# scttfrdmn/bwa-mem2-arm

Hardware: AMD Instinct MI355X
Metric: M seed-extensions/sec (150 bp, band=100) at 1/2/4/8 MI355X vs CPU (higher is better)
Workload: dtype int16; 1 GPU; C2: 1000000 SeqPairs/GPU resident in HBM, 150 bp query / 300 bp ref, band w=100, cell_bits=16, h0 U[19,100]; pairs_per_gpu=1000000, parallelism=shard1 (independent pairs), distinct_gpus=1

## Files before the change

bwa-mem2-arm_amd/csrc/bsw_dispatch.hip:

```cpp
#include <hip/hip_runtime.h>
#include <hipcub/hipcub.hpp>
#include <algorithm>
#include <cstring>
#include "bsw_engine.h"
#include <emmintrin.h>

namespace bsw {

constexpr int kNumLaneClasses = 5;
constexpr int kPkClass0 = kNumLaneClasses;
constexpr int kWideClass = kPkClass0 + kNumLaneClasses;
constexpr int kWvClass0 = kWideClass + 1;
constexpr int kNumWvClasses = 3;
constexpr int kWvCols[kNumWvClasses] = {4, 8, 16};
constexpr int kNumClasses = kWvClass0 + kNumWvClasses;
static_assert(kNumClasses <= kMetaCounts, "class counts");

__device__ __forceinline__ int seed_matches(const uint8_t *__restrict__ q, int qlen,
                                            const uint8_t *__restrict__ r, int tlen)
{
    if (qlen < 40 || tlen < 46) return 31;
    uint8_t qb[30], rb[42];
#pragma unroll
    for (int j = 0; j < 30; ++j) qb[j] = q[10 + j];
#pragma unroll
    for (int j = 0; j < 42; ++j) rb[j] = r[4 + j];
    int best = 0;
#pragma unroll
    for (int sft = 0; sft <= 12; ++sft) {
        int c = 0;
#pragma unroll
        for (int j = 0; j < 30; ++j) c += qb[j] == rb[j + sft];
        best = max(best, c);
    }
    return best;
}

__device__ __forceinline__ int wv_class(const KParams &kp, int32_t w, int qlen, int tlen, int h0)
{
    if (kp.maxsc != 1 || qlen > kWvQmax || h0 < 0) return -1;
    if ((int64_t)kp.e_ins * qlen >= 2700) return -1;
    if (128 + kp.o_del + 2 * kp.e_del >= 30000 || 128 + kp.o_ins + 2 * kp.e_ins >= 30000) return -1;
    if ((int64_t)h0 + min(qlen, tlen) + (int64_t)kp.e_ins * (qlen + 1) >= 30000) return -1;
    int wl = w;
    const int ni = qlen * kp.maxsc + kp.end_bonus - kp.o_ins;
    const int nd = qlen * kp.maxsc + kp.end_bonus - kp.o_del;
    wl = min(wl, max((ni + kp.e_ins) / kp.e_ins, 1));
    wl = min(wl, max((nd + kp.e_del) / kp.e_del, 1));
    for (int k = 0; k < kNumWvClasses; ++k)
        if (2 * wl + kWvCols[k] + 2 <= 64 * kWvCols[k]) return kWvClass0 + k;
    return -1;
}

__global__ void plan_kernel(const SeqPair *__restrict__ pairs, int32_t n, const KParams kp, int32_t w,
                            int32_t pc_route, int32_t wv_route, const uint8_t *__restrict__ ref,
                            const uint8_t *__restrict__ qer, uint32_t *__restrict__ keys,
                            int32_t *__restrict__ vals, int32_t *__restrict__ counts,
                            int32_t *__restrict__ maxq_wide, int keymode, int misroute)
{
    const int maxsc = kp.maxsc;
    const int i = blockIdx.x * blockDim.x + threadIdx.x;
    const bool valid = i < n;
    SeqPair p{};
    if (valid) p = pairs[i];
    const int qlen = max(p.len2, 0), tlen = max(p.len1, 0);
    const int64_t hi = (int64_t)max(p.h0, 0) + (int64_t)max(maxsc, 0) * min(qlen, tlen);
    int c = kWideClass;
    const int wvc = wv_route ? wv_class(kp, w, qlen, tlen, p.h0) : -1;
    if (wv_route == 2 && wvc >= 0) c = wvc;
    else if (hi < 32768 && p.h0 >= 0) {
        if (qlen <= 32) c = 0;
        else if (qlen <= 64) c = 1;
        else if (qlen <= 96) c = 2;
        else if (qlen <= 128) c = 3;
        else if (qlen <= 160) c = 4;
        if (pc_route && c < kNumLaneClasses && p.h0 + min(qlen, tlen) <= 255 && qlen + 1 <= 160)
            c = kPkClass0 + (qlen + 1 <= 32 ? 0 : qlen + 1 <= 64 ? 1 : qlen + 1 <= 96 ? 2 : qlen + 1 <= 128 ? 3 : 4);
    }
    if (c == kWideClass && wvc >= 0) c = wvc;
    if (misroute) c = 0;
    if (valid) {
        if (c == kWideClass) atomicMax(maxq_wide, qlen);
        const int mt = (c == kWideClass) ? 31 : seed_matches(qer + p.idq, qlen, ref + p.idr, tlen);
        const int rel = mt > 18;
        if (keymode == 0)
            keys[i] = ((uint32_t)c << 28) | ((uint32_t)(255 - min(qlen, 255)) << 20) |
                      ((uint32_t)(1 - rel) << 19) | ((uint32_t)(2047 - min(tlen, 2047)) << 8) |
                      (uint32_t)(255 - min(max(p.h0, 0), 255));
        else
            keys[i] = ((uint32_t)c << 28) | ((uint32_t)(255 - min(qlen, 255)) << 20) |
                      ((uint32_t)(1 - rel) << 19) | ((uint32_t)(63 - min(tlen >> 5, 63)) << 13) |
                      ((uint32_t)(31 - min(mt, 31)) << 8) | (uint32_t)(255 - min(max(p.h0, 0), 255));
        vals[i] = i;
    }
    __shared__ int s_cnt[kNumClasses];
    if (threadIdx.x < kNumClasses) s_cnt[threadIdx.x] = 0;
    __syncthreads();
    const int lane = threadIdx.x & 63;
#pragma unroll
// ... 126 lines not shown
        BSW_TRY(hipEventRecord(s.evh, pc.stream));
        BSW_TRY(hipStreamWaitEvent(stream, s.evh, 0));
    }
    BSW_TRY(grow_sort(s, n));
    BSW_TRY(hipMemsetAsync(s.d_meta, 0, kMetaWords * sizeof(int32_t), stream));
    int32_t *d_counts = s.d_meta, *d_maxq = s.d_meta + kMetaMaxq;
    const int pc_route = (kp.pk_ok && kp.kern8) ? 1 : 0;
    const int32_t long_route = (kp.long_route == 1 && n <= kp.small_batch) ? 2 : kp.long_route;
    hipLaunchKernelGGL(plan_kernel, dim3((unsigned)((n + 255) / 256)), dim3(256), 0, stream,
                       pc.d_pairs, n, kp, pc.w, pc_route, long_route, pc.d_ref, pc.d_qer, s.d_keys,
                       s.d_vals, d_counts, d_maxq, (int)kp.keymode, (int)kp.misroute);
    BSW_TRY(hipGetLastError());
    BSW_TRY(sort_order(s, n, kKeyBits, stream));
    BSW_TRY(hipMemcpyAsync(s.h_meta, s.d_meta, kMetaWords * sizeof(int32_t), hipMemcpyDeviceToHost, stream));
    if (!s.evm) BSW_TRY(hipEventCreateWithFlags(&s.evm.p, hipEventDisableTiming));
    BSW_TRY(hipEventRecord(s.evm, stream));
    return BSW_OK;
}

int run_dp(const KParams &kp, Slot &s)
{
    const PlanCall &pc = s.plan;
    if (pc.n == 0) return BSW_OK;
    hipStream_t stream = pc.dp_stream && !s.fast ? pc.dp_stream : pc.stream;
    const int32_t w = pc.w;
    const int cell_bits = pc.cell_bits;
    SeqPair *d_pairs = pc.d_pairs;
    const uint8_t *d_ref = pc.d_ref, *d_qer = pc.d_qer;
    int32_t *d_err = s.d_meta + kMetaErr;
    if (s.fast) {
        if (s.fast == 1) {
            BSW_TRY(hipEventSynchronize(s.evm));
            if (s.h_meta[kMetaFlag] != 0) {
                PlanCall again = pc;
                again.gq_maxq = -1;
                const int r = run_plan(kp, s, again);
                if (r) return r;
                return run_dp(kp, s);
            }
        }
        s.timed = true;
        return BSW_OK;
    }
    BSW_TRY(hipEventSynchronize(s.evm));
    BSW_TRY(hipStreamWaitEvent(stream, s.evm, 0));
    int32_t counts[kNumClasses] = {};
    for (int sl = 0; sl < kMetaSpread; ++sl)
        for (int c = 0; c < kNumClasses; ++c) counts[c] += s.h_meta[sl * kMetaCounts + c];
    const int32_t maxq_wide = s.h_meta[kMetaMaxq];
    int nclass = 0;
    for (int c = 0; c < kNumClasses; ++c) nclass += counts[c] > 0;
    const bool fork = nclass > 1 && kp.fork;
    BSW_TRY(hipEventRecord(s.ev0, stream));
    if (fork) {
        if (!s.evf) BSW_TRY(hipEventCreateWithFlags(&s.evf.p, hipEventDisableTiming));
        for (int k = 0; k < Slot::kSide; ++k)
            if (!s.side[k]) {
                BSW_TRY(hipStreamCreateWithFlags(&s.side[k].p, hipStreamNonBlocking));
                BSW_TRY(hipEventCreateWithFlags(&s.evj[k].p, hipEventDisableTiming));
            }
        BSW_TRY(hipEventRecord(s.evf, stream));
        for (int k = 0; k < Slot::kSide; ++k) BSW_TRY(hipStreamWaitEvent(s.side[k], s.evf, 0));
    }
    int nl = 0;
    auto next_stream = [&]() {
        const int k = nl++ % (1 + Slot::kSide);
        return (fork && k > 0) ? s.side[k - 1] : stream;
    };
    const int lrc = [&]() -> int {
        int32_t off = 0;
        for (int c = 0; c < kNumLaneClasses; ++c) {
            if (counts[c] > 0) {
                BSW_TRY(launch_lane_kernel(kLaneQmax[c], kp, w, d_pairs, s.d_order + off, counts[c],
                                           d_ref, d_qer, d_err, next_stream()));
                s.stats.n_launches++;
                s.stats.n_i16 += counts[c];
            }
            off += counts[c];
        }
        for (int c = 0; c < kNumLaneClasses; ++c) {
            const int32_t np = counts[kPkClass0 + c];
            if (np > 0) {
                BSW_TRY(launch_pc_kernel(kLaneQmax[c], kp, w, d_pairs, s.d_order + off, np, d_ref, d_qer,
                                         d_err, next_stream()));
                s.stats.n_launches++;
                s.stats.n_packed += np;
                if (cell_bits == 8) s.stats.n_u8 += np;
                else s.stats.n_i16 += np;
            }
            off += np;
        }
        if (counts[kWideClass] > 0) {
            const int32_t nw = counts[kWideClass];
            const size_t need = (size_t)(maxq_wide + 2) * (size_t)nw;
            BSW_TRY(s.d_scratch.grow(need));
            BSW_TRY(launch_wide_kernel(kp, w, d_pairs, s.d_order + off, nw, d_ref, d_qer, s.d_scratch,
                                       nw, next_stream()));
            s.stats.n_launches++;
            s.stats.n_wide += nw;
        }
        off += counts[kWideClass];
        for (int c = 0; c < kNumWvClasses; ++c) {
            const int32_t nv = counts[kWvClass0 + c];
            if (nv > 0) {
                BSW_TRY(launch_wv_kernel(kWvCols[c], kp, w, d_pairs, s.d_order + off, nv, d_ref, d_qer, d_err,
                                         next_stream()));
                s.stats.n_launches++;
                s.stats.n_i16 += nv;
                s.stats.n_wave += nv;
            }
            off += nv;
        }
        return BSW_OK;
    }();
    if (fork)
        for (int k = 0; k < Slot::kSide; ++k) {
            BSW_TRY(hipEventRecord(s.evj[k], s.side[k]));
            BSW_TRY(hipStreamWaitEvent(stream, s.evj[k], 0));
        }
    if (lrc) {
        (void)hipStreamSynchronize(stream);
        return lrc;
    }
    BSW_TRY(hipEventRecord(s.ev1, stream));
    BSW_TRY(hipMemcpyAsync(s.h_meta + kMetaErr, d_err, sizeof(int32_t), hipMemcpyDeviceToHost, stream));
    s.run_stream = stream;
    s.timed = true;
    return BSW_OK;
}

int run_device(const KParams &kp, Slot &s, SeqPair *d_pairs, const uint8_t *d_ref,
                      const uint8_t *d_qer, int32_t n, int32_t w, int cell_bits, hipStream_t stream)
{
    PlanCall pc;
    pc.d_pairs = d_pairs; pc.d_ref = d_ref; pc.d_qer = d_qer;
    pc.n = n; pc.w = w; pc.cell_bits = cell_bits; pc.stream = stream;
    int r = run_plan(kp, s, pc);
    if (r) return r;
    return run_dp(kp, s);
}

int finish_stats(Slot &s, bool spin)
{
    if (s.timed) {
        float ms = 0.f;
        s.timed = false;
        if (spin) {
            hipError_t q;
            while ((q = hipStreamQuery(s.run_stream)) == hipErrorNotReady) _mm_pause();
            BSW_TRY(q);
        }
        BSW_TRY(hipStreamSynchronize(s.run_stream));
        BSW_TRY(hipEventElapsedTime(&ms, s.ev0, s.ev1));
        s.stats.kernel_ms = ms;
        if (s.h_meta[kMetaErr] != 0) return BSW_E_RANGE;
    }
    return BSW_OK;
}

}
```

bwa-mem2-arm_amd/csrc/bsw_engine.h:

```cpp
#pragma once
#include <hip/hip_runtime.h>
#include <algorithm>
#include <atomic>
#include <condition_variable>
#include <cstdint>
#include <deque>
#include <memory>
#include <mutex>
#include <shared_mutex>
#include <type_traits>
#include <utility>
#include <vector>
#include "../../include/bsw.h"
#include "../../include/bsw_mate.h"
#include "../../include/bsw_global.h"
#include "../../include/bsw_aln.h"
#include "../../include/bsw_sel.h"
#include "../../include/bsw_pe.h"
#include "../../include/bsw_matesw.h"
#include "../../include/bsw_rec.h"
#include "../../include/bsw_contigs.h"
#include "bsw_contig_seg.h"
#include "bsw_kernels.h"
#include "bsw_internal.h"

#define BSW_HIDDEN __attribute__((visibility("hidden")))

namespace bsw {

constexpr int kMetaCounts = 16;
constexpr int kMetaSpread = 32;
constexpr int kMetaMaxq = kMetaCounts * kMetaSpread;
constexpr int kMetaErr = kMetaMaxq + 1;
constexpr int kMetaFlag = kMetaErr + 1;
constexpr int kMetaCnt = kMetaFlag + 1;
constexpr int kMetaWords = kMetaCnt + 1;
constexpr int kKeyBits = 32;
constexpr int32_t kStageBlk = 4096;

static inline int hip_rc(hipError_t e)
{
    if (e == hipSuccess) return BSW_OK;
    if (e == hipErrorOutOfMemory) return BSW_E_NOMEM;
    return BSW_E_HIP;
}
#define BSW_TRY(x) do { hipError_t _e = (x); if (_e != hipSuccess) return ::bsw::hip_rc(_e); } while (0)

BSW_HIDDEN bool inject_nomem();

template <class P, class Free>
struct BSW_HIDDEN Owned {
    P p = nullptr;
    Owned() = default;
    Owned(const Owned &) = delete;
    Owned &operator=(const Owned &) = delete;
    Owned(Owned &&o) noexcept : p(std::exchange(o.p, nullptr)) {}
    Owned &operator=(Owned &&o) noexcept { std::swap(p, o.p); return *this; }
    ~Owned() { reset(); }
    void reset() { if (p) (void)Free()(p); p = nullptr; }
    operator P() const { return p; }
};
struct BSW_HIDDEN FreeDev { hipError_t operator()(void *p) const { return hipFree(p); } };
struct BSW_HIDDEN FreeHost { hipError_t operator()(void *p) const { return hipHostFree(p); } };
struct BSW_HIDDEN FreeStream { hipError_t operator()(hipStream_t s) const { return hipStreamDestroy(s); } };
struct BSW_HIDDEN FreeEvent { hipError_t operator()(hipEvent_t e) const { return hipEventDestroy(e); } };
using Stream = Owned<hipStream_t, FreeStream>;
using Event = Owned<hipEvent_t, FreeEvent>;

template <class T, class Free>
struct BSW_HIDDEN Buf : Owned<T *, Free> {
    size_t cap = 0;
    Buf() = default;
    Buf(Buf &&o) noexcept : Owned<T *, Free>(std::move(o)), cap(std::exchange(o.cap, 0)) {}
    Buf &operator=(Buf &&o) noexcept { std::swap(this->p, o.p); std::swap(cap, o.cap); return *this; }
    void reset() { Owned<T *, Free>::reset(); cap = 0; }
    hipError_t reserve_exact(size_t n)
    {
        reset();
        hipError_t e;
        if constexpr (std::is_same<Free, FreeDev>::value) e = hipMalloc((void **)&this->p, n * sizeof(T));
        else e = hipHostMalloc((void **)&this->p, n * sizeof(T), 0);
        if (e == hipSuccess) cap = n;
        else this->p = nullptr;
        return e;
    }
    size_t grown(size_t need) const { return std::max(need + need / 4, cap * 3 / 2); }
};
template <class T>
struct BSW_HIDDEN DevBuf : Buf<T, FreeDev> {
    hipError_t grow(size_t need)
    {
        if (need <= this->cap) return hipSuccess;
        if (inject_nomem()) return hipErrorOutOfMemory;
        return this->reserve_exact(this->grown(need));
    }
};
template <class T>
struct BSW_HIDDEN PinnedBuf : Buf<T, FreeHost> {
    hipError_t grow(size_t need) { return need <= this->cap ? hipSuccess : this->reserve_exact(this->grown(need)); }
};

struct PlanCall {
    SeqPair *d_pairs = nullptr;
    const uint8_t *d_ref = nullptr, *d_qer = nullptr;
    int32_t n = 0, w = 0;
    int cell_bits = 16;
    hipStream_t stream = nullptr;
    hipStream_t dp_stream = nullptr;
    hipStream_t plan_stream = nullptr;
    int gq_maxq = -2, gq_maxt = 0;
    int32_t *d_out24 = nullptr;
};

struct ExtState;
struct AlnState;
struct SelW;
struct SelRd;
struct PeV;
struct MswSt;
// ... 262 lines not shown
```

bwa-mem2-arm_amd/csrc/bsw_kernels.h:

```cpp
#pragma once
#include <stdint.h>
#include <hip/hip_runtime.h>
#include "../../include/bsw_seqpair.h"

namespace bsw {

struct KParams {
    int32_t o_del, e_del, o_ins, e_ins;
    int32_t zdrop, end_bonus;
    int32_t maxsc;
    int32_t pk_ok;
    uint32_t prof[8][2];
    int8_t mat[25];
    int8_t kern8;
    int8_t keymode;
    int8_t fork;
    int8_t misroute;
    int8_t long_route;
    int8_t group_kernel;
    int32_t mid_batch;
    int32_t small_batch;
    int32_t gq32_max;
};

struct PairIn {
    int32_t idr, idq, len1, len2, h0;
};
static_assert(sizeof(PairIn) == 20, "PairIn");

constexpr int kLaneQmax[] = {32, 64, 96, 128, 160};
constexpr int kLaneQmaxMax = 160;

hipError_t launch_lane_kernel(int qmax, const KParams &kp, int32_t w, SeqPair *pairs,
                              const int32_t *order, int32_t n, const uint8_t *ref,
                              const uint8_t *qer, int32_t *err, hipStream_t s);

hipError_t launch_pc_kernel(int qmax, const KParams &kp, int32_t w, SeqPair *pairs,
                            const int32_t *order, int32_t n, const uint8_t *ref,
                            const uint8_t *qer, int32_t *err, hipStream_t s);

constexpr int kWvQmax = 4096;
hipError_t launch_wv_kernel(int cols, const KParams &kp, int32_t w, SeqPair *pairs, const int32_t *order,
                            int32_t n, const uint8_t *ref, const uint8_t *qer, int32_t *err, hipStream_t s);

hipError_t launch_gq_kernel(int gs, int cols, const KParams &kp, int32_t w, SeqPair *pairs, const int32_t *order,
                            int32_t n, const uint8_t *ref, const uint8_t *qer, int32_t *err, int32_t *flag,
                            int32_t *out24, hipStream_t s);
int gq_cols_for(int max_qlen, int gs);
bool gq_pair_ok(const KParams &kp, int qlen, int tlen, int h0, int gs);

hipError_t launch_wide_kernel(const KParams &kp, int32_t w, SeqPair *pairs,
                              const int32_t *order, int32_t n, const uint8_t *ref,
                              const uint8_t *qer, int2 *scratch, int32_t scratch_stride,
                              hipStream_t s);

}
```

bwa-mem2-arm_amd/csrc/bsw_pc.hip:

```cpp
#include <hip/hip_runtime.h>
#include <stdint.h>
#include <stdlib.h>
#include <limits.h>
#include <utility>
#include "bsw_kernels.h"
#include "bsw_wave.h"

namespace bsw {

constexpr int kPcChunkDw = 17;
#ifndef BSW_PC_EXP_HALFHEAD
#define BSW_PC_EXP_HALFHEAD 0
#endif
#ifdef BSW_PC_STATS
__device__ unsigned long long g_pc_stats[11];
constexpr int kPcTimesMax = 1 << 16;
__device__ unsigned long long g_pc_times[kPcTimesMax][4];
#endif

struct PcRow {
    uint64_t enter;
    uint64_t fast;
    uint64_t left;
};

__device__ __forceinline__ uint64_t gbits(int lo, int n)
{
    uint64_t m;
    asm("s_bfm_b64 %0, %1, %2" : "=s"(m)
        : "s"(__builtin_amdgcn_readfirstlane(min(n, 63))), "s"(__builtin_amdgcn_readfirstlane(lo)));
    return m;
}

__device__ __forceinline__ uint32_t pack2(int v) { return ((uint32_t)v & 0xffffu) * 0x10001u; }

#define PC_SDWA(op, d, a, b, sel) \
    op "_sdwa " d ", " a ", " b " dst_sel:DWORD dst_unused:UNUSED_PAD src0_sel:DWORD src1_sel:" sel "\n\t"

#define PC_PH1_(X, EOUT, ESUB)                                                          \
    "v_pk_min_i16 %[s" X "], %[s" X "], %[h" X "]\n\t"                                      \
    "v_pk_add_u16 %[s" X "], %[s" X "], %[h" X "]\n\t"                                      \
    "v_pk_sub_i16 %[t" X "], %[s" X "], %[oe2]\n\t"                                         \
    "v_pk_max_i16 %[s" X "], %[s" X "], %[e" X "]\n\t"                                      \
    ESUB                                                                                     \
    "v_pk_max_i16 " EOUT ", " EOUT ", %[t" X "]\n\t"
#define PC_PH1(X, EOUT) PC_PH1_(X, EOUT, "v_pk_sub_i16 " EOUT ", %[e" X "], %[ed2]\n\t")
#define PC_PH1B(X, EOUT) PC_PH1_(X, EOUT, "v_pk_sub_u16 " EOUT ", %[e" X "], %[ed2] clamp\n\t")

#define PC_SCORES                                                                        \
    "v_perm_b32 %[y], %[phi], %[plo], %[q]\n\t"                                              \
    "v_pk_lshlrev_b16 %[sa], 8, %[y] op_sel_hi:[0,1]\n\t"                                    \
    "v_pk_ashrrev_i16 %[sa], 8, %[sa] op_sel_hi:[0,1]\n\t"                                   \
    "v_pk_ashrrev_i16 %[sb], 8, %[y] op_sel_hi:[0,1]\n\t"

#define PC_CELL(C, X, W)                                                                 \
    PC_SDWA("v_max_i32", C, "%[f]", "sext(%[s" X "])", W)                                    \
    "v_subrev_u32_e64 %[f], %[ed], %[f] clamp\n\t"                                           \
    PC_SDWA("v_max_i32", "%[f]", "%[f]", "sext(%[t" X "])", W)

#define PC_RESET(HP, RJ)                                                                 \
    "v_cmp_ne_u32_e32 vcc, " RJ ", %[begv]\n\t"                                              \
    "v_cndmask_b32_e32 " HP ", 0, " HP ", vcc\n\t"                                           \
    "v_cndmask_b32_e32 %[f], 0, %[f], vcc\n\t"
#define PC_MCELL(C, HP, X, W, J)                                                         \
    PC_CELL(C, X, W)                                                                         \
    "v_cmp_lt_i32_e32 vcc, " J ", %[endv]\n\t"                                               \
    "v_cndmask_b32_e32 " C ", " HP ", " C ", vcc\n\t"

#define PC_MWRITE(X, KEYSRC, LEFT)                                                       \
    "v_pk_sub_i16 %[y], %[jj" X "], %[endw]\n\t"                                             \
    "v_pk_ashrrev_i16 %[y], 15, %[y] op_sel_hi:[0,1]\n\t"                                    \
    "v_bfi_b32 %[h" X "], %[y], %[p" X "], %[h" X "]\n\t"                                    \
    "v_bfi_b32 %[e" X "], %[y], 0, %[e" X "]\n\t"                                            \
    KEYSRC                                                                                   \
    "v_and_b32_e32 %[p" X "], %[p" X "], %[y]\n\t"                                           \
    "v_pk_sub_i16 %[y], %[jj" X "], %[endm1w]\n\t"                                           \
    "v_pk_ashrrev_i16 %[y], 15, %[y] op_sel_hi:[0,1]\n\t"                                    \
    "v_bfi_b32 %[e" X "], %[y], %[x" X "], %[e" X "]\n\t"                                    \
    LEFT                                                                                     \
    "v_pk_max_u16 %[key], %[key], %[p" X "]\n\t"
#define PC_LEFTMASK(X)                                                                   \
    "v_pk_sub_i16 %[y], %[begm2w], %[jj" X "]\n\t"                                           \
    "v_pk_ashrrev_i16 %[y], 15, %[y] op_sel_hi:[0,1]\n\t"                                    \
    "v_and_b32_e32 %[p" X "], %[p" X "], %[y]\n\t"

#define PC_MASKED(CH0, CH1, CH2, CH3, KA, KB, LA, LB) PC_MASKED_(PC_PH1, CH0, CH1, CH2, CH3, KA, KB, LA, LB)
#define PC_MASKED_(PH, CH0, CH1, CH2, CH3, KA, KB, LA, LB)                               \
    PH("a", "%[xa]") PH("b", "%[xb]")                                                        \
    CH0 CH1                                                                                  \
    "v_lshl_or_b32 %[pa], %[c0], 16, %[h1]\n\t"                                              \
    CH2 CH3                                                                                  \
    "v_lshl_or_b32 %[pb], %[c2], 16, %[c1]\n\t"                                              \
    PC_MWRITE("a", KA, LA) PC_MWRITE("b", KB, LB)

#ifdef BSW_PC_STATS
#define PC_CNT(k) "v_add_u32_e32 %[ct" #k "], 1, %[ct" #k "]\n\t"
#define PC_CNT_OPS , [ct0] "+v"(ctr[0]), [ct1] "+v"(ctr[1]), [ct2] "+v"(ctr[2]), [ct3] "+v"(ctr[3])
#else
// ... 345 lines not shown
        if constexpr (2 * GG + 1 < QMAX / 2) pc_lastpos_reg<2 * GG + 1>(hh[2 * GG + 1], endp1w, lp);
        pc_lastpos_reg<2 * GG>(hh[2 * GG], endp1w, lp);
    }
    return pending & (lp == 0u);
}

template <int QMAX, bool BY, int... G>
__device__ __forceinline__ int pc_lastpos(std::integer_sequence<int, G...>, const uint32_t (&hh)[(BY ? QMAX / 4 : QMAX / 2)],
                                          int end, bool need, int gstart)
{
    bool pending = need;
    uint32_t lp = 0;
    const uint32_t endp1w = pack2(end + 1);
    ((pending = pc_lastpos_group<QMAX, BY, QMAX / 4 - 1 - G>(hh, endp1w, pending, lp, gstart)), ...);
    return (int)max(lp & 0xffffu, lp >> 16);
}

#ifndef BSW_PC_EARLY_STOP
#define BSW_PC_EARLY_STOP 1
#endif
#ifndef BSW_PC_EARLY_SCAN
#define BSW_PC_EARLY_SCAN 1
#endif
#ifndef BSW_PC_SCAN_PHASE
#define BSW_PC_SCAN_PHASE 3
#endif

template <int K>
__device__ __forceinline__ void pc_ub_reg(uint32_t hv, uint32_t qw, uint32_t begw, uint32_t &ub)
{
    constexpr uint32_t SC = (uint32_t)(2 * K) | ((uint32_t)(2 * K + 1) << 16);
    uint32_t c, m;
    asm volatile(
        "v_pk_sub_i16 %[c], %[qw], %[sc]\n\t"
        "v_pk_ashrrev_i16 %[m], 15, %[c] op_sel_hi:[0,1]\n\t"
        "v_pk_add_u16 %[c], %[c], %[h]\n\t"
        "v_bfi_b32 %[c], %[m], 0, %[c]\n\t"
        "v_pk_sub_i16 %[m], %[bg], %[sc]\n\t"
        "v_pk_ashrrev_i16 %[m], 15, %[m] op_sel_hi:[0,1]\n\t"
        "v_and_b32_e32 %[c], %[c], %[m]\n\t"
        "v_pk_max_u16 %[ub], %[ub], %[c]\n\t"
        : [ub] "+v"(ub), [c] "=&v"(c), [m] "=&v"(m)
        : [h] "v"(hv), [qw] "v"(qw), [sc] "s"(SC), [bg] "v"(begw));
}

template <int QMAX, bool BY, int GG>
__device__ __forceinline__ void pc_ub_group(const uint32_t (&hh)[(BY ? QMAX / 4 : QMAX / 2)], uint32_t qw,
                                            uint32_t begw, uint32_t &ub, uint64_t enter)
{
    if (!((enter >> GG) & 1)) return;
    if constexpr (BY) {
        pc_ub_reg<2 * GG + 1>(__builtin_amdgcn_perm(hh[GG], hh[GG], kSelHi), qw, begw, ub);
        pc_ub_reg<2 * GG>(__builtin_amdgcn_perm(hh[GG], hh[GG], kSelLo), qw, begw, ub);
    } else {
        pc_ub_reg<2 * GG + 1>(hh[2 * GG + 1], qw, begw, ub);
        pc_ub_reg<2 * GG>(hh[2 * GG], qw, begw, ub);
    }
}

template <int QMAX, bool BY, int... G>
__device__ __forceinline__ int pc_ubscan(std::integer_sequence<int, G...>, const uint32_t (&hh)[(BY ? QMAX / 4 : QMAX / 2)],
                                         int qlen, int beg, uint64_t enter)
{
    uint32_t ub = 0;
    const uint32_t qw = pack2(qlen), begw = pack2(beg);
    (pc_ub_group<QMAX, BY, QMAX / 4 - 1 - G>(hh, qw, begw, ub, enter), ...);
    return (int)max(ub & 0xffffu, ub >> 16);
}

#ifndef BSW_PC_LEFT_SKIP
#define BSW_PC_LEFT_SKIP 1
#endif
#ifndef BSW_PC_SKIP_MASK
#define BSW_PC_SKIP_MASK 3
#endif
#ifndef BSW_PC_SKIP_ROW
#define BSW_PC_SKIP_ROW 1
#endif
#ifndef BSW_PC_SKIP_QMIN
#define BSW_PC_SKIP_QMIN 96
#endif
template <int QMAX> constexpr bool pc_left_skip() { return BSW_PC_LEFT_SKIP && QMAX >= BSW_PC_SKIP_QMIN; }

template <int QMAX, bool BY, int G>
__device__ __forceinline__ void pc_gz_group(const uint32_t (&hh)[(BY ? QMAX / 4 : QMAX / 2)],
                                            const uint32_t (&ee)[(BY ? QMAX / 4 : QMAX / 2)], bool live, int &gz)
{
    if constexpr (G < QMAX / 4) {
        if (gz != G) return;
        uint32_t z;
        if constexpr (BY) {
            asm volatile("v_or_b32_e32 %0, %1, %2" : "=v"(z) : "v"(hh[G]), "v"(ee[G]));
        } else {
            uint32_t t;
            asm volatile("v_pk_max_i16 %0, %2, 0\n\t"
                         "v_pk_max_i16 %1, %3, 0\n\t"
                         "v_or3_b32 %0, %0, %1, %4\n\t"
                         "v_or_b32_e32 %0, %0, %5"
                         : "=&v"(z), "=&v"(t)
                         : "v"(ee[2 * G]), "v"(ee[2 * G + 1]), "v"(hh[2 * G]), "v"(hh[2 * G + 1]));
        }
        if (__ballot(live && z != 0u) == 0) gz = G + 1;
    }
}

template <int QMAX, bool BY, int S, int... K>
__device__ __forceinline__ void pc_gz_seg(std::integer_sequence<int, K...>, const uint32_t (&hh)[(BY ? QMAX / 4 : QMAX / 2)],
                                          const uint32_t (&ee)[(BY ? QMAX / 4 : QMAX / 2)], bool live, int &gz)
{
    if ((gz >> 3) != S) return;
    (pc_gz_group<QMAX, BY, 8 * S + K>(hh, ee, live, gz), ...);
}

template <int QMAX, bool BY, int... S>
__device__ __forceinline__ void pc_gz_refresh(std::integer_sequence<int, S...>, const uint32_t (&hh)[(BY ? QMAX / 4 : QMAX / 2)],
                                              const uint32_t (&ee)[(BY ? QMAX / 4 : QMAX / 2)], bool live, int &gz)
{
    (pc_gz_seg<QMAX, BY, S>(std::make_integer_sequence<int, 8>{}, hh, ee, live, gz), ...);
}

template <int QMAX, int WPB, bool BY>
__global__ __launch_bounds__(64 * WPB, BY ? 3 : 2) void pc_kernel(const KParams kp, const int32_t w,
                                                    SeqPair *__restrict__ pairs,
                                                    const int32_t *__restrict__ order,
                                                    const int32_t n,
                                                    const uint8_t *__restrict__ ref,
                                                    const uint8_t *__restrict__ qer,
                                                    int32_t *__restrict__ err)
{
    constexpr int NG = QMAX / 4;
    constexpr int CDW = kPcChunkDw;
#ifdef BSW_PC_STATS
    const unsigned long long t_wave0 = wall_clock64();
#endif
    __shared__ uint32_t s_tgt[WPB][2][CDW][64];
    __shared__ uint2 s_prof[8];
    if (threadIdx.x < 8) s_prof[threadIdx.x] = make_uint2(kp.prof[threadIdx.x][0], kp.prof[threadIdx.x][1]);
    __syncthreads();
    const int gid = blockIdx.x * blockDim.x + threadIdx.x;
    bool valid = gid < n;
    const int idx = valid ? (order ? order[gid] : gid) : 0;
    SeqPair *sp = pairs + idx;
    int idr = 0, idq = 0, tlen = 0, qlen = 0, h0 = 0;
    if (valid) {
        idr = sp->idr; idq = sp->idq; tlen = sp->len1; qlen = sp->len2; h0 = sp->h0;
        if (qlen >= QMAX || qlen < 0 || tlen < 0 || h0 < 0 || h0 + min(qlen, tlen) > 255 || idr < 0 || idq < 0) {
            atomicOr(err, 1);
            valid = false;
        }
    }
    uint32_t qs[NG];
    {
        uint32_t wv[NG + 1];
        const uintptr_t qa = (uintptr_t)(qer + idq);
        const uint32_t *wp = (const uint32_t *)(qa & ~(uintptr_t)3);
        const int sh = (int)(qa & 3);
        const int nw = (valid && qlen > 0) ? (sh + qlen + 3) >> 2 : 0;
        if (nw > 0) {
#pragma unroll
            for (int g = 0; g <= NG; ++g) wv[g] = wp[min(g, nw - 1)];
        } else {
#pragma unroll
            for (int g = 0; g <= NG; ++g) wv[g] = 0;
        }
#pragma unroll
        for (int g = 0; g < NG; ++g) {
            const uint32_t c = __builtin_amdgcn_alignbyte(wv[g + 1], wv[g], sh);
            qs[g] = __builtin_amdgcn_perm(c, c, 0x03010200u);
        }
    }
    constexpr int NP = (BY ? QMAX / 4 : QMAX / 2);
    uint32_t hh[NP], ee[NP];
    {
        const int oe_ins = kp.o_ins + kp.e_ins;
        if constexpr (BY) {
            __builtin_amdgcn_sched_barrier(0);
#pragma unroll
            for (int k = 0; k < NP; ++k) {
                uint32_t v[4];
#pragma unroll
                for (int t = 0; t < 4; ++t) {
                    const int j = 4 * k + t;
                    v[t] = (j == 0) ? (uint32_t)h0 : (j <= qlen) ? (uint32_t)max(h0 - oe_ins - (j - 1) * kp.e_ins, 0) : 0u;
                }
                hh[k] = v[0] | (v[1] << 8) | (v[2] << 16) | (v[3] << 24);
                asm volatile("" : "+v"(hh[k]));
                ee[k] = 0u;
            }
        } else {
#pragma unroll
            for (int k = 0; k < NP; ++k) {
                const int j0 = 2 * k, j1 = 2 * k + 1;
                const uint32_t a = (j0 == 0) ? (uint32_t)h0
                                 : (j0 <= qlen) ? (uint32_t)max(h0 - oe_ins - (j0 - 1) * kp.e_ins, 0) : 0u;
                const uint32_t b = (j1 <= qlen) ? (uint32_t)max(h0 - oe_ins - (j1 - 1) * kp.e_ins, 0) : 0u;
                hh[k] = a | (b << 16);
                ee[k] = 0u;
            }
        }
    }
    int wl = w;
    {
        const int ni = qlen * kp.maxsc + kp.end_bonus - kp.o_ins;
        const int nd = qlen * kp.maxsc + kp.end_bonus - kp.o_del;
        wl = min(wl, max((ni + kp.e_ins) / kp.e_ins, 1));
        wl = min(wl, max((nd + kp.e_del) / kp.e_del, 1));
    }
    int best = h0, best_i = -1, best_j = -1, max_ie = -1, gsc = -1, moff = 0, endc = qlen;
    bool alive = valid && tlen > 0;
    if (!valid) sp = nullptr;
    asm volatile("" : "+v"(sp));
    const uint8_t *tp = ref + idr;
    const int tsh = (int)((uintptr_t)tp & 3);
    const uint32_t *twp = (const uint32_t *)(tp - tsh);
    const int tlast = max((tsh + tlen - 1) >> 2, 0);
    const int wv = threadIdx.x >> 6, ln = threadIdx.x & 63;
    auto issue_chunk = [&](int ch) {
        uint32_t *dst = &s_tgt[wv][ch & 1][0][0];
#pragma unroll
        for (int k = 0; k < CDW; ++k)
            __builtin_amdgcn_global_load_lds((gptr_t)(twp + min(16 * ch + k, tlast)),
                                             (lptr_t)(dst + 64 * k), 4, 0, 0);
    };
    if (alive) { issue_chunk(0); issue_chunk(1); }
    uint32_t tcur = 0;
    const int wl_max = wave_max(alive ? wl : -1);
    const int wl_min = wave_min(alive ? wl : INT_MAX);
    const uint32_t oe2 = (uint32_t)(kp.o_del + kp.e_del) * 0x10001u;
    const uint32_t ed2 = (uint32_t)kp.e_del * 0x10001u;
    uint32_t ctr[4] = {0, 0, 0, 0};
    PcbSel bs{BY ? kSelKa : 0x06010400u, BY ? kSelKb : 0x06030402u};
    if constexpr (BY || (BSW_PC_JKEY && QMAX >= 128)) asm volatile("" : "+v"(bs.ka), "+v"(bs.kb));
#ifdef BSW_PC_STATS
    uint32_t nrows = 0, nlast = 0, nue = 0;
    uint32_t nscan = 0, nstop_s = 0, nstop_c = 0;
    (void)nscan; (void)nstop_s; (void)nstop_c;
#endif

#if BSW_PC_EXP_HALFHEAD
    int emax = 0, emin = 0;
    PcRow r{0, 0, 0};
#endif
    int gz = 0;
    (void)gz;
    for (int i = 0;; ++i) {
        const bool act = alive && i < tlen;
        alive = act;
        if (__ballot(act) == 0) break;
        if ((i & 3) == 0) {
            if ((i & 63) == 0) {
                __builtin_amdgcn_s_waitcnt(0x0F70);
                __builtin_amdgcn_sched_barrier(0);
            }
            const int k = (i >> 2) & 15;
            const uint32_t la = (uint32_t)(uintptr_t)(lptr_t)&s_tgt[wv][(i >> 6) & 1][k][ln];
            uint2 d;
            asm volatile("ds_read2st64_b32 %0, %1 offset1:1\n\ts_waitcnt lgkmcnt(0)"
                         : "=v"(d) : "v"(la) : "memory");
            tcur = __builtin_amdgcn_alignbyte(d.y, d.x, tsh);
            if ((i & 63) == 0) {
                __builtin_amdgcn_sched_barrier(0);
                if (i > 0 && act) issue_chunk((i >> 6) + 1);
            }
        }
        const uint32_t tcode = (tcur >> (8 * (i & 3))) & 0xffu;
        const uint2 pr = s_prof[min(tcode, 7u)];
        __builtin_amdgcn_sched_barrier(0);
        const int beg = max(0, i - wl);
        const int end = min(min(endc, i + wl + 1), qlen);
        endc = end;
#if BSW_PC_EXP_HALFHEAD
        if (i & 1) goto row_body;
#else
        int emax, emin;
        PcRow r;
#endif
        wave_maxmin_bc(act ? end : -1, act ? end : INT_MAX, emax, emin);
        {
            const int ulo = __builtin_amdgcn_readfirstlane(max(0, i - wl_max));
            const int uhi = __builtin_amdgcn_readfirstlane(emax);
            const int flo = __builtin_amdgcn_readfirstlane(max(0, i - wl_min));
            const int fhi = __builtin_amdgcn_readfirstlane(emin);
            const int glo = ulo >> 2;
            const int gsp = max((min(uhi, QMAX - 1) >> 2) - glo, -1);
            const int gfa = (ulo == flo && (flo & 3) == 0) ? (flo >> 2) : (flo >> 2) + 1;
            const int gfn = max((fhi >> 2) - gfa, 0);
            const int gln = (flo >> 2) - glo;
            r.enter = gbits(glo, gsp + 1);
            r.fast = gbits(gfa, gfn);
            r.left = gbits(glo, gln + 1);
            if constexpr (pc_left_skip<QMAX>()) {
                const uint64_t keep = ~0ull << gz;
                r.enter &= keep;
                r.fast &= keep;
            }
        }
#if BSW_PC_EXP_HALFHEAD
    row_body:
#endif
        {
            int h1 = (int)((uint32_t)max(h0 - (kp.o_del + kp.e_del * (i + 1)), 0) << 16) & -(int)(beg == 0);
            int f = 0;
            uint32_t key = 0;
            const uint32_t endw = pack2(end);
            const uint32_t endm1w = pack2(end - 1);
            const uint32_t begm2w = pack2(beg - 2);
            __builtin_amdgcn_s_setprio(0);
            pc_row<QMAX, BY>(std::make_integer_sequence<int, (NG + pc_seg_len<QMAX>() - 1) / pc_seg_len<QMAX>()>{}, hh, ee,
                             qs, pr.x, pr.y, f, h1, key, oe2, ed2, kp.e_del, r, endw, endm1w, begm2w, end, beg, bs,
                             ctr);
            __builtin_amdgcn_s_setprio(2);
            h1 = (int)((uint32_t)h1 >> 16);
            const uint32_t k32 = max(key & 0xffffu, key >> 16);
            const int m = (int)(k32 >> 8), mj = (int)(k32 & 0xffu);
            {
                const bool atq = act && end == qlen;
                max_ie = (atq && !(gsc > h1)) ? i : max_ie;
                gsc = atq ? max(gsc, h1) : gsc;
            }
            {
                const int di = i - best_i, dj = mj - best_j;
                const int dz = (di > dj) ? best - m - (int)__umul24((unsigned)(di - dj), (unsigned)kp.e_del)
                                         : best - m - (int)__umul24((unsigned)(dj - di), (unsigned)kp.e_ins);
                const bool better = act && m > best;
                const bool zdropped = kp.zdrop > 0 && dz > kp.zdrop;
                alive = act && m > 0 && (better || !zdropped);
                moff = better ? max(moff, abs(mj - i)) : moff;
                best_i = better ? i : best_i;
                best_j = better ? mj : best_j;
                best = better ? m : best;
            }
#if BSW_PC_EARLY_STOP
            {
                int gq, gt, gm;
                asm volatile("v_sub_u32_e32 %0, %3, %4\n\t"
                             "v_subrev_u32_e32 %1, %5, %6\n\t"
                             "v_sub_u32_e32 %2, %3, %7"
                             : "=&v"(gq), "=&v"(gt), "=&v"(gm)
                             : "v"(qlen), "v"(beg), "s"(i), "v"(tlen), "v"(mj));
                const bool edge = end == qlen && gq < qlen;
                const int ubs = m - 1 + min(gq, gt);
                const bool stop = edge && ubs <= best && ubs < gsc;
#ifdef BSW_PC_STATS
                nstop_s += alive && stop;
#endif
                alive = alive && !stop;
#if BSW_PC_EARLY_SCAN
                const int ubm = m - 1 + gm;
                const bool want = QMAX > 64 && alive && edge && ubm <= best && ubm < gsc;
                if (QMAX > 64 && (i & BSW_PC_SCAN_PHASE) == BSW_PC_SCAN_PHASE && __ballot(want)) {
                    const int ubc = pc_ubscan<QMAX, BY>(std::make_integer_sequence<int, NG>{}, hh, gq + beg, beg, r.enter);
                    const bool stopc = want && ubc <= best && ubc < gsc;
#ifdef BSW_PC_STATS
                    nscan += 1;
                    nstop_c += stopc;
#endif
                    alive = alive && !stopc;
                }
#endif
            }
#endif
            if constexpr (pc_left_skip<QMAX>()) {
                if ((i & BSW_PC_SKIP_MASK) == BSW_PC_SKIP_ROW)
                    pc_gz_refresh<QMAX, BY>(std::make_integer_sequence<int, (NG + 7) / 8>{}, hh, ee, alive, gz);
            }
#ifdef BSW_PC_STATS
            nrows += act;
            nue += act && (emax == emin);
#endif
            {
                const bool need = alive && h1 == 0;
                int lp1 = end;
                if (__ballot(need)) {
#ifdef BSW_PC_STATS
                    nlast += 1;
#endif
                    const int lp = pc_lastpos<QMAX, BY>(std::make_integer_sequence<int, NG>{}, hh, end, need,
                                                        emax >> 2);
                    lp1 = need ? lp : end;
                }
                endc = alive ? min(lp1 + 2, qlen) : endc;
            }
        }
    }
#ifdef BSW_PC_STATS
    {
        const unsigned rows = (unsigned)wave_max((int)nrows);
        const unsigned nl = (unsigned)wave_max((int)nlast);
        const unsigned nu = (unsigned)wave_max((int)nue);
        const unsigned ns = (unsigned)wave_max((int)nscan);
        const unsigned rs = (unsigned)__popcll(__ballot(nstop_s != 0));
        const unsigned rc = (unsigned)__popcll(__ballot(nstop_c != 0));
        unsigned cmax[4];
        for (int k = 0; k < 4; ++k) cmax[k] = (unsigned)wave_max((int)ctr[k]);
        if ((threadIdx.x & 63) == 0) {
            atomicAdd(&g_pc_stats[0], (unsigned long long)rows);
            for (int k = 0; k < 4; ++k) atomicAdd(&g_pc_stats[1 + k], (unsigned long long)cmax[k]);
            atomicAdd(&g_pc_stats[5], (unsigned long long)nl);
            atomicAdd(&g_pc_stats[6], 1ull);
            atomicAdd(&g_pc_stats[7], (unsigned long long)nu);
            atomicAdd(&g_pc_stats[8], (unsigned long long)ns);
            atomicAdd(&g_pc_stats[9], (unsigned long long)rs);
            atomicAdd(&g_pc_stats[10], (unsigned long long)rc);
        }
        const unsigned wid = blockIdx.x * WPB + (threadIdx.x >> 6);
        if ((threadIdx.x & 63) == 0 && wid < (unsigned)kPcTimesMax) {
            unsigned xcc, hw;
            asm volatile("s_getreg_b32 %0, hwreg(HW_REG_XCC_ID)" : "=s"(xcc));
            asm volatile("s_getreg_b32 %0, hwreg(HW_REG_HW_ID)" : "=s"(hw));
            g_pc_times[wid][0] = t_wave0;
            g_pc_times[wid][1] = wall_clock64();
            g_pc_times[wid][2] = ((unsigned long long)xcc << 32) | hw;
            g_pc_times[wid][3] = rows;
        }
    }
#endif
    if (sp) {
        sp->score = best;
        sp->tle = best_i + 1;
        sp->gtle = max_ie + 1;
        sp->qle = best_j + 1;
        sp->gscore = gsc;
        sp->max_off = moff;
    }
}

#ifdef BSW_PC_STATS
extern "C" int bsw_pc_stats(unsigned long long *out, int reset)
{
    if (hipMemcpyFromSymbol(out, HIP_SYMBOL(g_pc_stats), 11 * sizeof(unsigned long long)) != hipSuccess) return -5;
    if (reset) {
        unsigned long long z[11] = {0, 0, 0, 0, 0, 0, 0, 0, 0, 0, 0};
        if (hipMemcpyToSymbol(HIP_SYMBOL(g_pc_stats), z, sizeof(z)) != hipSuccess) return -5;
    }
    return 0;
}
extern "C" int bsw_pc_times(unsigned long long *out, int n)
{
    n = n < kPcTimesMax ? n : kPcTimesMax;
    if (hipMemcpyFromSymbol(out, HIP_SYMBOL(g_pc_times), (size_t)n * 32) != hipSuccess) return -5;
    return n;
}
#endif

template <int QMAX>
static void launch_pc_q(const KParams &kp, int32_t w, SeqPair *pairs, const int32_t *order, int32_t n,
                        const uint8_t *ref, const uint8_t *qer, int32_t *err, hipStream_t s)
{
    const unsigned grid = (unsigned)((n + 63) / 64);
    if (kp.kern8 == 2)
        hipLaunchKernelGGL((pc_kernel<QMAX, 1, true>), dim3(grid), dim3(64), 0, s, kp, w, pairs, order, n,
                           ref, qer, err);
    else
        hipLaunchKernelGGL((pc_kernel<QMAX, 1, false>), dim3(grid), dim3(64), 0, s, kp, w, pairs, order,
                           n, ref, qer, err);
}

hipError_t launch_pc_kernel(int qmax, const KParams &kp, int32_t w, SeqPair *pairs,
                            const int32_t *order, int32_t n, const uint8_t *ref,
                            const uint8_t *qer, int32_t *err, hipStream_t s)
{
    if (n <= 0) return hipSuccess;
    switch (qmax) {
    case 32: launch_pc_q<32>(kp, w, pairs, order, n, ref, qer, err, s); break;
    case 64: launch_pc_q<64>(kp, w, pairs, order, n, ref, qer, err, s); break;
    case 96: launch_pc_q<96>(kp, w, pairs, order, n, ref, qer, err, s); break;
    case 128: launch_pc_q<128>(kp, w, pairs, order, n, ref, qer, err, s); break;
    case 160: launch_pc_q<160>(kp, w, pairs, order, n, ref, qer, err, s); break;
    default: return hipErrorInvalidValue;
    }
    return hipGetLastError();
}

}
```

Measured before the change: 180.1 M seed-extensions/s.

## Prune dominated left column groups in packed kernel with exact redo pass

After: 186.1 M seed-extensions/s, median of 6. +3.3%, better.

```diff
diff --git a/bwa-mem2-arm_amd/csrc/bsw_dispatch.hip b/bwa-mem2-arm_amd/csrc/bsw_dispatch.hip
--- a/bwa-mem2-arm_amd/csrc/bsw_dispatch.hip
+++ b/bwa-mem2-arm_amd/csrc/bsw_dispatch.hip
@@ -15,6 +15,7 @@
 constexpr int kWvCols[kNumWvClasses] = {4, 8, 16};
 constexpr int kNumClasses = kWvClass0 + kNumWvClasses;
 static_assert(kNumClasses <= kMetaCounts, "class counts");
+static_assert(kNumLaneClasses <= kMetaRedoWords && kMetaRedo + kMetaRedoWords <= kMetaWords, "redo-list lengths");
 
 __device__ __forceinline__ int seed_matches(const uint8_t *__restrict__ q, int qlen,
                                             const uint8_t *__restrict__ r, int tlen)
@@ -307,7 +308,8 @@
             const int32_t np = counts[kPkClass0 + c];
             if (np > 0) {
                 BSW_TRY(launch_pc_kernel(kLaneQmax[c], kp, w, d_pairs, s.d_order + off, np, d_ref, d_qer,
-                                         d_err, next_stream()));
+                                         d_err, reinterpret_cast<int32_t *>(s.d_keys2.p) + off,
+                                         s.d_meta + kMetaRedo + c, next_stream()));
                 s.stats.n_launches++;
                 s.stats.n_packed += np;
                 if (cell_bits == 8) s.stats.n_u8 += np;
diff --git a/bwa-mem2-arm_amd/csrc/bsw_engine.h b/bwa-mem2-arm_amd/csrc/bsw_engine.h
--- a/bwa-mem2-arm_amd/csrc/bsw_engine.h
+++ b/bwa-mem2-arm_amd/csrc/bsw_engine.h
@@ -34,7 +34,9 @@
 constexpr int kMetaErr = kMetaMaxq + 1;
 constexpr int kMetaFlag = kMetaErr + 1;
 constexpr int kMetaCnt = kMetaFlag + 1;
-constexpr int kMetaWords = kMetaCnt + 1;
+constexpr int kMetaRedo = kMetaCnt + 1;
+constexpr int kMetaRedoWords = 5;
+constexpr int kMetaWords = kMetaRedo + kMetaRedoWords;
 constexpr int kKeyBits = 32;
 constexpr int32_t kStageBlk = 4096;
 
diff --git a/bwa-mem2-arm_amd/csrc/bsw_kernels.h b/bwa-mem2-arm_amd/csrc/bsw_kernels.h
--- a/bwa-mem2-arm_amd/csrc/bsw_kernels.h
+++ b/bwa-mem2-arm_amd/csrc/bsw_kernels.h
@@ -37,7 +37,7 @@
 
 hipError_t launch_pc_kernel(int qmax, const KParams &kp, int32_t w, SeqPair *pairs,
                             const int32_t *order, int32_t n, const uint8_t *ref,
-                            const uint8_t *qer, int32_t *err, hipStream_t s);
+                            const uint8_t *qer, int32_t *err, int32_t *redo, int32_t *rcnt, hipStream_t s);
 
 constexpr int kWvQmax = 4096;
 hipError_t launch_wv_kernel(int cols, const KParams &kp, int32_t w, SeqPair *pairs, const int32_t *order,
diff --git a/bwa-mem2-arm_amd/csrc/bsw_pc.hip b/bwa-mem2-arm_amd/csrc/bsw_pc.hip
--- a/bwa-mem2-arm_amd/csrc/bsw_pc.hip
+++ b/bwa-mem2-arm_amd/csrc/bsw_pc.hip
@@ -13,7 +13,7 @@
 #define BSW_PC_EXP_HALFHEAD 0
 #endif
 #ifdef BSW_PC_STATS
-__device__ unsigned long long g_pc_stats[11];
+__device__ unsigned long long g_pc_stats[13];
 constexpr int kPcTimesMax = 1 << 16;
 __device__ unsigned long long g_pc_times[kPcTimesMax][4];
 #endif
@@ -525,12 +525,59 @@
 #endif
 template <int QMAX> constexpr bool pc_left_skip() { return BSW_PC_LEFT_SKIP && QMAX >= BSW_PC_SKIP_QMIN; }
 
-template <int QMAX, bool BY, int G>
-__device__ __forceinline__ void pc_gz_group(const uint32_t (&hh)[(BY ? QMAX / 4 : QMAX / 2)],
-                                            const uint32_t (&ee)[(BY ? QMAX / 4 : QMAX / 2)], bool live, int &gz)
+#ifndef BSW_PC_LEFT_PRUNE
+#define BSW_PC_LEFT_PRUNE 1
+#endif
+#ifndef BSW_PC_PRUNE_QMIN
+#define BSW_PC_PRUNE_QMIN 128
+#endif
+template <int QMAX, bool BY> constexpr bool pc_left_prune()
+{
+    return BSW_PC_LEFT_PRUNE && !BY && pc_left_skip<QMAX>() && QMAX >= BSW_PC_PRUNE_QMIN;
+}
+#ifndef BSW_PC_PRUNE_BRANCH
+#define BSW_PC_PRUNE_BRANCH 1
+#endif
+constexpr int kPcPruned = 1 << 8;
+template <bool PRUNE> __device__ __forceinline__ int pc_gz_of(int gz) { return PRUNE ? (gz & (kPcPruned - 1)) : gz; }
+
+template <int K>
+__device__ __forceinline__ void pc_pb_reg(uint32_t v, uint32_t gw, uint32_t bw, uint32_t &ub)
+{
+    constexpr uint32_t SC = (uint32_t)(2 * K) | ((uint32_t)(2 * K + 1) << 16);
+    uint32_t c, m;
+    asm volatile(
+        "v_pk_sub_i16 %[c], %[gw], %[sc]\n\t"
+        "v_pk_min_u16 %[m], %[v], 1 op_sel_hi:[1,0]\n\t"
+        "v_pk_mul_lo_u16 %[c], %[c], %[m]\n\t"
+        "v_pk_add_u16 %[c], %[c], %[v]\n\t"
+        "v_pk_sub_i16 %[m], %[bw], %[sc]\n\t"
+        "v_pk_ashrrev_i16 %[m], 15, %[m] op_sel_hi:[0,1]\n\t"
+        "v_and_b32_e32 %[c], %[c], %[m]\n\t"
+        "v_pk_max_u16 %[ub], %[ub], %[c]\n\t"
+        : [ub] "+v"(ub), [c] "=&v"(c), [m] "=&v"(m)
+        : [v] "v"(v), [gw] "v"(gw), [sc] "s"(SC), [bw] "v"(bw));
+}
+
+__device__ __forceinline__ uint32_t pc_pos2(uint32_t e)
+{
+    uint32_t r;
+    asm volatile("v_pk_max_i16 %0, %1, 0" : "=v"(r) : "v"(e));
+    return r;
+}
+
+struct PcPrune {
+    bool pre;
+    int qlen, beg, gsc;
+    uint32_t npr;
+};
+
+template <int QMAX, bool BY, bool PRUNE, int G>
+__device__ __forceinline__ void pc_gz_group(uint32_t (&hh)[(BY ? QMAX / 4 : QMAX / 2)],
+                                            uint32_t (&ee)[(BY ? QMAX / 4 : QMAX / 2)], bool live, int &gz, PcPrune &pp)
 {
     if constexpr (G < QMAX / 4) {
-        if (gz != G) return;
+        if (pc_gz_of<PRUNE>(gz) != G) return;
         uint32_t z;
         if constexpr (BY) {
             asm volatile("v_or_b32_e32 %0, %1, %2" : "=v"(z) : "v"(hh[G]), "v"(ee[G]));
@@ -543,34 +590,57 @@
                          : "=&v"(z), "=&v"(t)
                          : "v"(ee[2 * G]), "v"(ee[2 * G + 1]), "v"(hh[2 * G]), "v"(hh[2 * G + 1]));
         }
-        if (__ballot(live && z != 0u) == 0) gz = G + 1;
-    }
-}
-
-template <int QMAX, bool BY, int S, int... K>
-__device__ __forceinline__ void pc_gz_seg(std::integer_sequence<int, K...>, const uint32_t (&hh)[(BY ? QMAX / 4 : QMAX / 2)],
-                                          const uint32_t (&ee)[(BY ? QMAX / 4 : QMAX / 2)], bool live, int &gz)
-{
-    if ((gz >> 3) != S) return;
-    (pc_gz_group<QMAX, BY, 8 * S + K>(hh, ee, live, gz), ...);
-}
-
-template <int QMAX, bool BY, int... S>
-__device__ __forceinline__ void pc_gz_refresh(std::integer_sequence<int, S...>, const uint32_t (&hh)[(BY ? QMAX / 4 : QMAX / 2)],
-                                              const uint32_t (&ee)[(BY ? QMAX / 4 : QMAX / 2)], bool live, int &gz)
-{
-    (pc_gz_seg<QMAX, BY, S>(std::make_integer_sequence<int, 8>{}, hh, ee, live, gz), ...);
-}
-
-template <int QMAX, int WPB, bool BY>
+        if (__ballot(live && z != 0u) == 0) {
+            gz = PRUNE ? gz + 1 : G + 1;
+        } else if constexpr (PRUNE) {
+            if (!pp.pre) return;
+            uint32_t ub = 0;
+            const uint32_t qw = pack2(pp.qlen), qm1w = pack2(pp.qlen - 1);
+            const uint32_t bgw = pack2(pp.beg), bgm1w = pack2(pp.beg - 1);
+            static_assert(!BY, "the byte planes are compiled without the prune");
+            pc_pb_reg<2 * G + 1>(hh[2 * G + 1], qw, bgw, ub);
+            pc_pb_reg<2 * G>(hh[2 * G], qw, bgw, ub);
+            pc_pb_reg<2 * G + 1>(pc_pos2(ee[2 * G + 1]), qm1w, bgm1w, ub);
+            pc_pb_reg<2 * G>(pc_pos2(ee[2 * G]), qm1w, bgm1w, ub);
+            const int u = (int)max(ub & 0xffffu, ub >> 16);
+            if (__ballot(live && u >= pp.gsc) == 0) {
+                hh[2 * G] = 0u; hh[2 * G + 1] = 0u; ee[2 * G] = 0u; ee[2 * G + 1] = 0u;
+                gz = (G + 1) | kPcPruned;
+#ifdef BSW_PC_STATS
+                pp.npr += 1;
+#endif
+            }
+        }
+    }
+}
+
+template <int QMAX, bool BY, bool PRUNE, int S, int... K>
+__device__ __forceinline__ void pc_gz_seg(std::integer_sequence<int, K...>, uint32_t (&hh)[(BY ? QMAX / 4 : QMAX / 2)],
+                                          uint32_t (&ee)[(BY ? QMAX / 4 : QMAX / 2)], bool live, int &gz, PcPrune &pp)
+{
+    if ((pc_gz_of<PRUNE>(gz) >> 3) != S) return;
+    (pc_gz_group<QMAX, BY, PRUNE, 8 * S + K>(hh, ee, live, gz, pp), ...);
+}
+
+template <int QMAX, bool BY, bool PRUNE, int... S>
+__device__ __forceinline__ void pc_gz_refresh(std::integer_sequence<int, S...>, uint32_t (&hh)[(BY ? QMAX / 4 : QMAX / 2)],
+                                              uint32_t (&ee)[(BY ? QMAX / 4 : QMAX / 2)], bool live, int &gz, PcPrune &pp)
+{
+    (pc_gz_seg<QMAX, BY, PRUNE, S>(std::make_integer_sequence<int, 8>{}, hh, ee, live, gz, pp), ...);
+}
+
+template <int QMAX, int WPB, bool BY, bool REDO>
 __global__ __launch_bounds__(64 * WPB, BY ? 3 : 2) void pc_kernel(const KParams kp, const int32_t w,
                                                     SeqPair *__restrict__ pairs,
                                                     const int32_t *__restrict__ order,
-                                                    const int32_t n,
+                                                    const int32_t n_in,
                                                     const uint8_t *__restrict__ ref,
                                                     const uint8_t *__restrict__ qer,
-                                                    int32_t *__restrict__ err)
-{
+                                                    int32_t *__restrict__ err,
+                                                    int32_t *__restrict__ redo,
+                                                    int32_t *__restrict__ rcnt)
+{
+    constexpr bool PRUNE = !REDO && pc_left_prune<QMAX, BY>();
     constexpr int NG = QMAX / 4;
     constexpr int CDW = kPcChunkDw;
 #ifdef BSW_PC_STATS
@@ -578,6 +648,11 @@
 #endif
     __shared__ uint32_t s_tgt[WPB][2][CDW][64];
     __shared__ uint2 s_prof[8];
+    int32_t n = n_in;
+    if constexpr (REDO) {
+        n = min(n, *rcnt);
+        if ((int)(blockIdx.x * blockDim.x) >= n) return;
+    }
     if (threadIdx.x < 8) s_prof[threadIdx.x] = make_uint2(kp.prof[threadIdx.x][0], kp.prof[threadIdx.x][1]);
     __syncthreads();
     const int gid = blockIdx.x * blockDim.x + threadIdx.x;
@@ -686,6 +761,7 @@
 #endif
     int gz = 0;
     (void)gz;
+    PcPrune pp{false, 0, 0, 0, 0u};
     for (int i = 0;; ++i) {
         const bool act = alive && i < tlen;
         alive = act;
@@ -733,7 +809,7 @@
             r.fast = gbits(gfa, gfn);
             r.left = gbits(glo, gln + 1);
             if constexpr (pc_left_skip<QMAX>()) {
-                const uint64_t keep = ~0ull << gz;
+                const uint64_t keep = ~0ull << pc_gz_of<PRUNE>(gz);
                 r.enter &= keep;
                 r.fast &= keep;
             }
@@ -772,6 +848,18 @@
                 best_i = better ? i : best_i;
                 best_j = better ? mj : best_j;
                 best = better ? m : best;
+                if constexpr (PRUNE) {
+#if BSW_PC_PRUNE_BRANCH
+                    if (gz & kPcPruned)
+#endif
+                    {
+                        const bool rd = (gz & kPcPruned) != 0 &&
+                                        ((act && !better && m > 0 && kp.zdrop > 0 && best - m > kp.zdrop) ||
+                                         (alive && h1 == 0));
+                        alive = alive && !rd;
+                        sp = (SeqPair *)((uintptr_t)sp | (uintptr_t)rd);
+                    }
+                }
             }
 #if BSW_PC_EARLY_STOP
             {
@@ -804,8 +892,15 @@
             }
 #endif
             if constexpr (pc_left_skip<QMAX>()) {
-                if ((i & BSW_PC_SKIP_MASK) == BSW_PC_SKIP_ROW)
-                    pc_gz_refresh<QMAX, BY>(std::make_integer_sequence<int, (NG + 7) / 8>{}, hh, ee, alive, gz);
+                if ((i & BSW_PC_SKIP_MASK) == BSW_PC_SKIP_ROW) {
+                    if constexpr (PRUNE) {
+                        pp.pre = i > wl_max && __ballot(alive && !(end == qlen && gsc > 0)) == 0;
+                        asm volatile("v_mov_b32_e32 %0, %1" : "=v"(pp.qlen) : "v"(qlen));
+                        pp.beg = beg; pp.gsc = gsc;
+                    }
+                    pc_gz_refresh<QMAX, BY, PRUNE>(std::make_integer_sequence<int, (NG + 7) / 8>{}, hh, ee, alive, gz,
+                                                   pp);
+                }
             }
 #ifdef BSW_PC_STATS
             nrows += act;
@@ -858,6 +953,26 @@
         }
     }
 #endif
+    if constexpr (PRUNE) {
+        const bool rd = ((uintptr_t)sp & 1u) != 0;
+        const unsigned long long rb = __ballot(rd);
+        if (rb) {
+            int base = 0;
+            if (ln == __ffsll((long long)rb) - 1) base = atomicAdd(rcnt, (int)__popcll(rb));
+            base = __shfl(base, __ffsll((long long)rb) - 1);
+            if (rd) {
+                const unsigned g = blockIdx.x * blockDim.x + threadIdx.x;
+                redo[base + (int)__popcll(rb & ((1ull << ln) - 1ull))] = order ? order[g] : (int)g;
+            }
+        }
+#ifdef BSW_PC_STATS
+        if (ln == 0) {
+            atomicAdd(&g_pc_stats[11], (unsigned long long)pp.npr);
+            atomicAdd(&g_pc_stats[12], (unsigned long long)__popcll(rb));
+        }
+#endif
+        if (rd) sp = nullptr;
+    }
     if (sp) {
         sp->score = best;
         sp->tle = best_i + 1;
@@ -871,9 +986,9 @@
 #ifdef BSW_PC_STATS
 extern "C" int bsw_pc_stats(unsigned long long *out, int reset)
 {
-    if (hipMemcpyFromSymbol(out, HIP_SYMBOL(g_pc_stats), 11 * sizeof(unsigned long long)) != hipSuccess) return -5;
+    if (hipMemcpyFromSymbol(out, HIP_SYMBOL(g_pc_stats), 13 * sizeof(unsigned long long)) != hipSuccess) return -5;
     if (reset) {
-        unsigned long long z[11] = {0, 0, 0, 0, 0, 0, 0, 0, 0, 0, 0};
+        unsigned long long z[13] = {0, 0, 0, 0, 0, 0, 0, 0, 0, 0, 0, 0, 0};
         if (hipMemcpyToSymbol(HIP_SYMBOL(g_pc_stats), z, sizeof(z)) != hipSuccess) return -5;
     }
     return 0;
@@ -888,28 +1003,37 @@
 
 template <int QMAX>
 static void launch_pc_q(const KParams &kp, int32_t w, SeqPair *pairs, const int32_t *order, int32_t n,
-                        const uint8_t *ref, const uint8_t *qer, int32_t *err, hipStream_t s)
+                        const uint8_t *ref, const uint8_t *qer, int32_t *err, int32_t *redo, int32_t *rcnt,
+                        hipStream_t s)
 {
     const unsigned grid = (unsigned)((n + 63) / 64);
     if (kp.kern8 == 2)
-        hipLaunchKernelGGL((pc_kernel<QMAX, 1, true>), dim3(grid), dim3(64), 0, s, kp, w, pairs, order, n,
-                           ref, qer, err);
+        hipLaunchKernelGGL((pc_kernel<QMAX, 1, true, false>), dim3(grid), dim3(64), 0, s, kp, w, pairs, order, n,
+                           ref, qer, err, redo, rcnt);
     else
-        hipLaunchKernelGGL((pc_kernel<QMAX, 1, false>), dim3(grid), dim3(64), 0, s, kp, w, pairs, order,
-                           n, ref, qer, err);
+        hipLaunchKernelGGL((pc_kernel<QMAX, 1, false, false>), dim3(grid), dim3(64), 0, s, kp, w, pairs, order,
+                           n, ref, qer, err, redo, rcnt);
+    if constexpr (pc_left_prune<QMAX, false>()) {
+        constexpr int kRedoWpb = 4;
+        const unsigned rgrid = (unsigned)((n + 64 * kRedoWpb - 1) / (64 * kRedoWpb));
+        if (kp.kern8 != 2)
+            hipLaunchKernelGGL((pc_kernel<QMAX, kRedoWpb, false, true>), dim3(rgrid), dim3(64 * kRedoWpb), 0, s, kp, w,
+                               pairs, redo, n, ref, qer, err, nullptr, rcnt);
+    }
 }
 
 hipError_t launch_pc_kernel(int qmax, const KParams &kp, int32_t w, SeqPair *pairs,
                             const int32_t *order, int32_t n, const uint8_t *ref,
-                            const uint8_t *qer, int32_t *err, hipStream_t s)
+                            const uint8_t *qer, int32_t *err, int32_t *redo, int32_t *rcnt, hipStream_t s)
 {
     if (n <= 0) return hipSuccess;
+    if (!redo || !rcnt) return hipErrorInvalidValue;
     switch (qmax) {
-    case 32: launch_pc_q<32>(kp, w, pairs, order, n, ref, qer, err, s); break;
-    case 64: launch_pc_q<64>(kp, w, pairs, order, n, ref, qer, err, s); break;
-    case 96: launch_pc_q<96>(kp, w, pairs, order, n, ref, qer, err, s); break;
-    case 128: launch_pc_q<128>(kp, w, pairs, order, n, ref, qer, err, s); break;
-    case 160: launch_pc_q<160>(kp, w, pairs, order, n, ref, qer, err, s); break;
+    case 32: launch_pc_q<32>(kp, w, pairs, order, n, ref, qer, err, redo, rcnt, s); break;
+    case 64: launch_pc_q<64>(kp, w, pairs, order, n, ref, qer, err, redo, rcnt, s); break;
+    case 96: launch_pc_q<96>(kp, w, pairs, order, n, ref, qer, err, redo, rcnt, s); break;
+    case 128: launch_pc_q<128>(kp, w, pairs, order, n, ref, qer, err, redo, rcnt, s); break;
+    case 160: launch_pc_q<160>(kp, w, pairs, order, n, ref, qer, err, redo, rcnt, s); break;
     default: return hipErrorInvalidValue;
     }
     return hipGetLastError();
```
